# Amandaynzhou/MMT-PSM

Measured on AMD Instinct MI355X. Metric: imgs/sec (student+teacher step, 1000x1000, AUG_K=2), higher is better.
Workload: dtype f32

## Files before the change

### include/mmtpsm.h

```cpp
#ifndef MMTPSM_H
#define MMTPSM_H
#include <stdint.h>
#ifdef __cplusplus
extern "C" {
#endif

#define MMT_EINVAL (-22)

int mmt_version(void);

typedef struct {
  const float* feat[4];
  float* grad_feat[4];
  int H[4];
  int W[4];
  float scale[4];
  int num_levels;
  int N;
  int C;
} mmt_pyramid;

int mmt_roi_align_forward(const mmt_pyramid* pyr , const float* rois, const int32_t* levels,
                          int K, int PH, int PW, int sampling_ratio, float* out, void* stream);
int mmt_roi_align_forward_bf16(const mmt_pyramid* pyr , const float* rois, const int32_t* levels,
// ... 103 lines not shown
  const void* f16_guard_x;
  const void* f16_guard_dy;
  const void* w_src;
  const void* w_src_scale;
  int x_planes_layout;
  void* y_rb;
  long y_rb_stride;
  const float* y_rb_scale;
  void* y_amax_next;
  int x_planes_lag;
  int y_rb_rows;
} mmt_conv_args;

int mmt_conv_forward(const mmt_conv_args* a , void* stream);
int mmt_conv_variant(const mmt_conv_args* a );
int mmt_conv_ksplit(const mmt_conv_args* a );
int mmt_conv_wants_planes(const mmt_conv_args* a );
int mmt_set_conv_precision(int mode);
int mmt_amax(const float* x, long n, const float* rowscale, long inner, int rows, float* amax , void* stream);
int mmt_amax_stats(const float* x, long n, float* slot , void* stream);
int mmt_sum_stats(const float* a, const float* b, const float* c, const float* d, float* y, long n,
                  float* slot , void* stream);
int mmt_stats_combine(const float* const* slots , int n, float* out , void* stream);
int mmt_split_planes_f16(const float* x, void* planes, long plane_stride, long n, float scale, const float* amax ,
                         float* scale_out , float* amax_next ,
                         float* zero_slot , void* stream);
int mmt_pack_weight_f16(const float* w, void* planes, long plane_stride, int Cout, int K, float scale, const float* amax,
                        float* scale_out, void* stream);
int mmt_pack_weight_flipped_f16(const float* w, const float* scale, void* planes, long plane_stride, int Cout, int KH, int KW,
                                int Cin, const float* amax, float* scale_out, void* stream);
int mmt_conv3x3_strip_f16x2(const mmt_conv_args* a , const float* s_x , const float* s_w , void* stream);
int mmt_conv_forward_f16x2(const mmt_conv_args* a , const float* x_amax , const float* s_w , void* stream);
int mmt_get_conv_precision(void);
int mmt_stem_fused(const float* x, int N, int H, int W, const float* w_s2d, const void* w_planes, long w_plane_stride,
                   const float* s_w , const float* scale, const float* shift, const float* x_slot , float* y,
                   float* y_slot , void* stream);
int mmt_conv_wgrad_planes_splits(const mmt_conv_args* a );
int mmt_conv_wgrad_planes(const mmt_conv_args* a , const float* dy, const void* x_planes, long x_plane_stride,
                          const void* dy_planes, long dy_plane_stride, const float* s_x, const float* s_dy, const float* rowscale,
                          float* dw, float* dbias, float* workspace, void* stream);
typedef struct {
  void* fn;
  long a[16];
} mmt_call;
int mmt_replay(const mmt_call* calls , int n, int* failed_index );
int mmt_split_planes_f16_rb(const float* x, void* planes, long plane_stride, int rows, int W, int C, const float* amax,
                            float* scale_out, void* stream);
int mmt_conv_writes_rb(const mmt_conv_args* a );
typedef struct mmt_wgrad_job {
  mmt_conv_args a;
  const float* dy; const float* rowscale; float* dw; float* dbias;
  const void* x_planes; long x_plane_stride; const void* dy_planes; long dy_plane_stride; const float* s_x; const float* s_dy;
} mmt_wgrad_job;
int mmt_conv_wgrad_group_workspace(const mmt_wgrad_job* jobs , int n, long* floats_out );
int mmt_conv_wgrad_group(const mmt_wgrad_job* jobs , int n, float* workspace, long workspace_floats, void* stream);
int mmt_sum_stats_rb(const float* a, const float* b, const float* c, const float* d, float* y, int rows, int W, int C, float* slot,
                     void* planes, long plane_stride, const float* scale, float* amax_next, void* stream);
int mmt_rb_scales_update(float* state, int n, void* stream);
int mmt_conv_forward_pg(const mmt_conv_args* a , const float* s_x , const float* s_w , int tile_rows,
                        int ksplit, void* stream);
int mmt_conv_pg_plan(const mmt_conv_args* a , int* tile_rows, int* ksplit);
int mmt_conv_pg_wanted(const mmt_conv_args* a );
typedef struct { long src_off, dst_off; int Cout, K, unit0, pad; } mmt_pack_desc;
long mmt_packed_weight_elems(int Cout, int K);
int mmt_pack_weight(const float* w, void* planes, long plane_stride, int Cout, int K, void* stream);
int mmt_pack_weight_flipped(const float* w, const float* scale, void* planes, long plane_stride, int Cout, int KH, int KW,
// ... 110 lines not shown
```

### mmt-psm_amd/csrc/conv_igemm.hip

```cpp
#include <stdlib.h>
#include <map>
#include <mutex>
#include <type_traits>
#include "conv_shared.h"

namespace {

template <int BM, int BN, int WM, int WN>
__device__ __forceinline__ void conv_epilogue_stage(f32x16 (&acc)[BM / (32 * WM)][BN / (32 * WN)], float* lds,
                                                    const int lane, const int wm, const int wn) {
  constexpr int TM = BM / (32 * WM), TN = BN / (32 * WN);
  float* ct = lds;
  const int col_l = lane & 31, rq = lane >> 5;
#pragma unroll
  for (int a = 0; a < TM; a++)
#pragma unroll
    for (int b = 0; b < TN; b++)
#pragma unroll
      for (int r = 0; r < 16; r++) {
        const int row = (wm * TM + a) * 32 + (r & 3) + 8 * (r >> 2) + 4 * rq;
        ct[row * BN + (wn * TN + b) * 32 + col_l] = acc[a][b][r];
      }
}

// ... 125 lines not shown
            for (int e = 0; e < 4; e++) { const float av = e < nv ? fabsf(v[e]) : 0.f; amx = fmaxf(amx, av); asum += av; }
            acnt += (float)nv;
          }
          if (p.io & IO_Y) {
            unsigned short* yh = (unsigned short*)p.y + oidx[g];
            const unsigned lo = pk_bf16(v[0], v[1]), hi = pk_bf16(v[2], v[3]);
            if (vec) *(uint2*)yh = uint2{lo, hi};
            else { const unsigned short h4[4] = {(unsigned short)lo, (unsigned short)(lo >> 16), (unsigned short)hi, (unsigned short)(hi >> 16)};
                   for (int e = 0; e < nv; e++) yh[e] = h4[e]; }
            continue;
          }
          if (vec) *(f32x4*)(p.y + oidx[g]) = f32x4{v[0], v[1], v[2], v[3]};
          else for (int e = 0; e < nv; e++) p.y[oidx[g] + e] = v[e];
          if (p.ypl) {
            uint2 o[3];
            split4<3>(f32x4{v[0], v[1], v[2], v[3]}, o);
#pragma unroll
            for (int q = 0; q < 3; q++) *(uint2*)(p.ypl + q * p.ypl_stride + oidx[g]) = o[q];
          }
          if (p.yrb && m0 + r0 + (g0 + g) * RPP < p.yrb_M) rb_store4(p, rbg, m0 + r0 + (g0 + g) * RPP, c, f32x4{v[0], v[1], v[2], v[3]}, rbs);
        }
      }
    }
  }
  if (p.amax_out) {
    if (acc) { acc->amx = fmaxf(acc->amx, amx); acc->asum += asum; acc->acnt += acnt; }
    else conv_amax_commit(p, AmaxAcc{amx, asum, acnt}, blockIdx.x);
  }
}

template <int BM, int BN, int WM, int WN>
__device__ __forceinline__ void conv_epilogue(const ConvP& p, f32x16 (&acc)[BM / (32 * WM)][BN / (32 * WN)], float* lds,
                                              const int m0, const int n0, const int tid, const int lane,
                                              const int wm, const int wn, const int HoWo) {
  conv_epilogue_stage<BM, BN, WM, WN>(acc, lds, lane, wm, wn);
  __syncthreads();
  conv_epilogue_finish<BM, BN>(p, lds, m0, n0, tid, HoWo);
}

template <int BM, int BN, int WM, int WN>
__global__ __launch_bounds__(256, 2) void conv_fwd_kernel(const ConvP p) {
  constexpr int TM = BM / (32 * WM), TN = BN / (32 * WN);
  constexpr int NA = BM / 32, NB = BN / 32;
  extern __shared__ __attribute__((aligned(16))) float lds[];
  float* ldsA = lds;
  float* ldsB = lds + 2 * BM * 32;

  const int tid = threadIdx.x;
  const int lane = tid & 63;
  const int wave = __builtin_amdgcn_readfirstlane(tid >> 6);
  const int wm = wave / WN, wn = wave % WN;

  const int tiles_m = (p.M + BM - 1) / BM;
  const int tiles_n = (p.Cout + BN - 1) / BN;
  int bid = blockIdx.x;
  {
    const int nwg = tiles_m * tiles_n, q = nwg >> 3, r = nwg & 7, xcd = bid & 7, idx = bid >> 3;
    bid = (xcd < r ? xcd * (q + 1) : r * (q + 1) + (xcd - r) * q) + idx;
  }
  const int tile_m = bid / tiles_n, tile_n = bid % tiles_n;
  const int m0 = tile_m * BM, n0 = tile_n * BN;

  const int c4 = tid & 7;
  const int r8 = tid >> 3;
  unsigned abase[NA];
  int aih0[NA], aiw0[NA];
  bool aok[NA];
  const int HoWo = p.Ho * p.Wo;
#pragma unroll
  for (int j = 0; j < NA; j++) {
// ... 253 lines not shown
#pragma unroll
      for (int b = 0; b < TN; b++) fb[q][b] = *(const bf16x8*)(B + q * PB + b * 32 * 32);
    }
#pragma unroll
    for (int sum = 2 * (NS - 1) > NS - 1 ? NS - 1 : 0; sum >= 0; sum--)
#pragma unroll
      for (int qa = 0; qa <= sum; qa++) {
        const int qb = sum - qa;
        if (qa < NS && qb < NS) {
#pragma unroll
          for (int a = 0; a < TM; a++)
#pragma unroll
            for (int b = 0; b < TN; b++)
              acc[a][b] = __builtin_amdgcn_mfma_f32_32x32x16_bf16(fa[qa][a], fb[qb][b], acc[a][b], 0, 0, 0);
        }
      }
    if (kt + 1 < nkt) store_tile(buf ^ 1);
    __syncthreads();
  }
  conv_epilogue<BM, BN, WM, WN>(p, acc, lds, m0, n0, tid, lane, wm, wn, HoWo);
}

__device__ __attribute__((aligned(16))) const float g_zero16[4] = {0.f, 0.f, 0.f, 0.f};

__device__ __forceinline__ void dma16(const void* g, void* l) {
  __builtin_amdgcn_global_load_lds((const __attribute__((address_space(1))) void*)g, (lds_ptr_t)l, 16, 0, 0);
}

__device__ __forceinline__ void dma16_unseen(const void* g, void* l) {
#if defined(__HIP_DEVICE_COMPILE__)
  const unsigned la = __builtin_amdgcn_readfirstlane((unsigned)(unsigned long)(__attribute__((address_space(3))) char*)l);
  asm volatile("s_mov_b32 m0, %1\n\ts_nop 0\n\tglobal_load_lds_dwordx4 %0, off" ::"v"(g), "s"(la) : "m0", "memory");
#endif
}

template <int BM, int BN, int WM, int WN, int NS, int S, bool F16 = false>
__global__ __launch_bounds__(256, 2) void conv_fwd_glds_kernel(const ConvP p, const unsigned short* __restrict__ wpl,
                                                               const long wpl_stride, const int ksplit,
                                                               float* __restrict__ ws) {
  constexpr int TM = BM / (32 * WM), TN = BN / (32 * WN);
  constexpr int A_BYTES = BM * 64;
  constexpr int PB = BN * 32;
  constexpr int STAGE = A_BYTES + NS * PB;
  constexpr int NIA = BM / 64;
  constexpr int NIB_TOT = NS * BN / 32;
  constexpr int NIB = (NIB_TOT + 3) / 4;
  constexpr int NI = NIA + NIB;
  extern __shared__ __attribute__((aligned(16))) float lds[];
  char* const ring = (char*)lds;

  const int tid = threadIdx.x;
  const int lane = tid & 63;
  const int wave = __builtin_amdgcn_readfirstlane(tid >> 6);
  const int wm = wave / WN, wn = wave % WN;

  const int tiles_m = (p.M + BM - 1) / BM;
  const int tiles_n = (p.Cout + BN - 1) / BN;
  int bid = blockIdx.x;
  {
    const int nwg = tiles_m * tiles_n * ksplit, q = nwg >> 3, r = nwg & 7, xcd = bid & 7, idx = bid >> 3;
    bid = (xcd < r ? xcd * (q + 1) : r * (q + 1) + (xcd - r) * q) + idx;
  }
  const int ks = bid % ksplit;
  bid /= ksplit;
  const int tile_m = bid / tiles_n, tile_n = bid % tiles_n;
  const int m0 = tile_m * BM, n0 = tile_n * BN;
  const int HoWo = p.Ho * p.Wo;
  F16Guard guard = {};
  if constexpr (F16) guard = f16_guard_load(p.guard_x);
  unsigned abase[NIA];
  int aih0[NIA], aiw0[NIA], achunk[NIA];
  bool aok[NIA];
#pragma unroll
  for (int i = 0; i < NIA; i++) {
    const int row = (wave + 4 * i) * 16 + (lane >> 2);
    const int m = m0 + row;
    aok[i] = m < p.M;
    const int mm = aok[i] ? m : 0;
    const int img = mm / HoWo, rem = mm - img * HoWo;
    const int ho = rem / p.Wo, wo = rem - ho * p.Wo;
    aih0[i] = ho * p.stride - p.pad;
    aiw0[i] = wo * p.stride - p.pad;
    abase[i] = (unsigned)img * (unsigned)(p.H * p.W * p.Cin);
    achunk[i] = ((lane & 3) ^ ((row >> 2) & 3)) * 4;
  }
  const int nb32 = (p.Cout + 31) >> 5;
  const long kt_stride = (long)nb32 * 512;
  const unsigned short* bsrc[NIB];
  int bdst[NIB];
#pragma unroll
  for (int i = 0; i < NIB; i++) {
    const int t = (wave + 4 * i) % NIB_TOT;
    const int q = t / (BN / 32), rb = t % (BN / 32);
    int nb = n0 / 32 + rb;
    if (nb >= nb32) nb = nb32 - 1;
    bsrc[i] = wpl + q * wpl_stride + (long)nb * 512 + lane * 8;
    bdst[i] = A_BYTES + q * PB + rb * 1024;
  }
// ... 129 lines not shown
    __builtin_amdgcn_s_barrier();
    tap_next();
    filling = kt + S < nkt;
    const int kt_fill = min(kt + S, nkt - 1);
    constexpr int NM = TM * TN * (NS * (NS + 1) / 2);
    int j = 0, mi = 0;
#pragma unroll
    for (int sum = NS - 1; sum >= 0; sum--)
#pragma unroll
      for (int qa = 0; qa <= sum; qa++) {
        const int qb = sum - qa;
#pragma unroll
        for (int a = 0; a < TM; a++)
#pragma unroll
          for (int b = 0; b < TN; b++) {
            if constexpr (F16)
              acc[a][b] = __builtin_amdgcn_mfma_f32_32x32x16_f16(__builtin_bit_cast(f16x8, fa[qa][a]), __builtin_bit_cast(f16x8, fb[qb][b]), acc[a][b], 0, 0, 0);
            else
              acc[a][b] = __builtin_amdgcn_mfma_f32_32x32x16_bf16(fa[qa][a], fb[qb][b], acc[a][b], 0, 0, 0);
            j++;
#pragma unroll
            for (int r = 0; r < (NMICRO + NM - 1) / NM; r++)
              if (mi < (j * NMICRO + NM - 1) / NM) { micro(mi, kt_fill, stage_free, stage_next, fan, fbn); mi++; }
            __builtin_amdgcn_sched_barrier(0);
          }
      }
  };
#pragma unroll
  for (int t = 0; t < S - 1; t++) { filling = t < nkt; issue_all(min(t, nkt - 1), t); }
  if constexpr (F16) {
    if (f16_guard_bad(guard)) {
      asm volatile("s_waitcnt vmcnt(0)" ::: "memory");
      float* slab = ksplit > 1 ? ws + ((long)bid * ksplit + ks) * (BM * BN) : nullptr;
      conv_slow_tile(m0, BM, 0, BM, n0, BN, slab, ks != 0, tid, 256, blockIdx.x);
      return;
    }
  }
  wait_dma(S - 2);
  __builtin_amdgcn_s_barrier();
  filling = S - 1 < nkt;
  issue_all(min(S - 1, nkt - 1), S - 1);
  bf16x8 fa0[NS][TM], fb0[NS][TN], fa1[NS][TM], fb1[NS][TN];
  {
    const char* st = ring;
#pragma unroll
    for (int a = 0; a < TM; a++) { va[a][0] = *(const f32x4*)(st + aoff[a][0]); va[a][1] = *(const f32x4*)(st + aoff[a][1]); }
#pragma unroll
    for (int q = 0; q < NS; q++)
#pragma unroll
      for (int b = 0; b < TN; b++) fb0[q][b] = *(const bf16x8*)(st + boff + q * PB + b * 1024);
#pragma unroll
    for (int lvl = 0; lvl < SPL; lvl++)
#pragma unroll
      for (int f = 0; f < 2 * TM; f++) { if (lvl & 1) split_sub(f >> 1, f & 1); else split_cvt(f >> 1, f & 1, lvl >> 1); }
    pack_a(fa0);
  }
  int stage = 0;
  for (int kt = 0; kt < nkt; kt += 2) {
    const int s1 = stage == S - 1 ? 0 : stage + 1, s2 = s1 == S - 1 ? 0 : s1 + 1;
    step(kt, s1, stage, fa0, fb0, fa1, fb1);
    if (kt + 1 < nkt) step(kt + 1, s2, s1, fa1, fb1, fa0, fb0);
    stage = s2;
  }
  asm volatile("s_waitcnt vmcnt(0)" ::: "memory");
  __syncthreads();
  if (ksplit == 1) {
    if (!p.staged_epilogue && !p.io && !p.ypl && !p.mul && p.res_mode <= 1 && p.out_stride == 1 && (long)p.M * p.Cout * 4 < (1L << 31)) {
      const int mrow0 = m0 + wm * TM * 32 + 4 * (lane >> 5);
      conv_epilogue_direct<TM, TN>(p, acc, (unsigned)mrow0 * ((unsigned)p.Cout * 4u), p.M - mrow0, n0 + wn * TN * 32 + (lane & 31),
                                   (1 << (TM * TN)) - 1, lds + 64, wave, lane, tid, blockIdx.x);
      return;
    }
    conv_epilogue<BM, BN, WM, WN>(p, acc, lds, m0, n0, tid, lane, wm, wn, HoWo);
    return;
  }
  conv_epilogue_stage<BM, BN, WM, WN>(acc, lds, lane, wm, wn);
  __syncthreads();
  constexpr int TILE4 = BM * BN / 4;
  f32x4* slab = (f32x4*)ws + ((long)bid * ksplit + ks) * TILE4;
  const f32x4* ct4 = (const f32x4*)lds;
  for (int i = tid; i < TILE4; i += 256) slab[i] = ct4[i];
}

template <int BM, int BN, int WM, int WN, int NS, int S>
__global__ __launch_bounds__(256, 2) void conv_fwd_pp_kernel(const ConvP p, const int ksplit, float* __restrict__ ws) {
  constexpr int TM = BM / (32 * WM), TN = BN / (32 * WN);
  constexpr int PA = BM * 32, PB = BN * 32;
  constexpr int A_BYTES = NS * PA;
  constexpr int STAGE = A_BYTES + NS * PB;
  constexpr int NIA_TOT = NS * BM / 32, NIB_TOT = NS * BN / 32;
  constexpr int NIA = (NIA_TOT + 3) / 4, NIB = (NIB_TOT + 3) / 4, NI = NIA + NIB;
  static_assert(BM / 32 == 4 || BM / 32 == 2, "row blocks per wave");
  extern __shared__ __attribute__((aligned(16))) float lds[];
  char* const ring = (char*)lds;

  const int tid = threadIdx.x;
  const int lane = tid & 63;
  const int wave = __builtin_amdgcn_readfirstlane(tid >> 6);
  const int wm = wave / WN, wn = wave % WN;

  const int tiles_m = (p.M + BM - 1) / BM;
  const int tiles_n = (p.Cout + BN - 1) / BN;
  int bid = blockIdx.x;
  {
    const int nwg = tiles_m * tiles_n * ksplit, q = nwg >> 3, r = nwg & 7, xcd = bid & 7, idx = bid >> 3;
    bid = (xcd < r ? xcd * (q + 1) : r * (q + 1) + (xcd - r) * q) + idx;
// ... 1015 lines not shown
  }
}

template <int NS>
int launch_split_variant(int variant, const ConvP& p, hipStream_t s) {
  switch (variant) {
    case 1: return launch_split<128, 128, 2, 2, NS>(p, s);
    case 3: return launch_split<128, 64, 2, 2, NS>(p, s);
    default: return launch_split<64, 64, 2, 2, NS>(p, s);
  }
}

}

namespace mmtconv {
static int g_precision = -1;
int precision() {
  if (g_precision < 0) {
    g_precision = getenv("MMT_CONV_PRECISION") ? atoi(getenv("MMT_CONV_PRECISION")) : 3;
    if (g_precision < 0 || g_precision > 3) g_precision = 3;
  }
  return g_precision;
}
}

extern "C" int mmt_set_conv_precision(int mode) {
  if (mode < 0 || mode > 3) return MMT_EINVAL;
  mmtconv::g_precision = mode;
  return 0;
}

extern "C" int mmt_get_conv_precision(void) { return precision(); }

extern "C" int mmt_conv3x3_strip_f16x2(const mmt_conv_args* a, const float* s_x, const float* s_w, void* stream) {
  ConvP p;
  int e = fill(p, a);
  if (e) return e;
  if (!p.y || !p.xpl || !p.wpl || !s_x || !s_w || p.io || p.ypl) return MMT_EINVAL;
  p.f16_sx = s_x; p.f16_sw = s_w;
  const int tw = strip_tw(p);
  if (!tw) return MMT_EINVAL;
  const int ksplit = strip_ksplit(p, tw);
  constexpr int NS = 2;
  hipStream_t s = (hipStream_t)stream;
  SplitWs w{nullptr, nullptr};
  if (ksplit > 1) {
    w = split_workspace(s);
    if (!w.ws) return MMT_EINVAL;
  }
  const int tiles = p.N * (p.Ho * p.Wo / 256) * mmt_cdiv(p.Cout, 128);
  auto go = [&](auto kern, int TW) {
    const int R = 256 / TW, SW = TW + 32;
    const size_t ring = (size_t)2 * (NS * R * SW * 32 + 3 * NS * 128 * 32), epi = (size_t)256 * 128 * sizeof(float);
    const size_t lds = ring > epi ? ring : epi;
    const hipError_t er = hipFuncSetAttribute((const void*)kern, hipFuncAttributeMaxDynamicSharedMemorySize, (int)lds);
    if (er != hipSuccess) return (int)er;
    hipLaunchKernelGGL(kern, dim3(tiles * ksplit), dim3(512), lds, s, p, ksplit | strip_korder(p), w.ws);
    return 0;
  };
  if (tw == 128) e = go(conv3x3_strip_kernel<128, NS, true>, 128);
  else e = go(conv3x3_strip_kernel<64, NS, true>, 64);
  if (e) return e;
  MMT_LAUNCH_CHECK();
  if (ksplit > 1) {
    launch_finish<256, 128>(p, tiles, ksplit, w.ws, s);
    MMT_LAUNCH_CHECK();
// ... 8 lines not shown
  return true;
}
extern "C" int mmt_conv_writes_rb(const mmt_conv_args* a) {
  ConvP p;
  if (fill(p, a) || precision() != 3 || p.io) return 0;
  p.f16_ax = 1;
  p.f16_sx = p.f16_sw = (const float*)16;
  return rb_epilogue_ok(p) ? 1 : 0;
}
extern "C" int mmt_conv_forward_f16x2(const mmt_conv_args* a, const float* x_amax, const float* s_w, void* stream) {
  ConvP p;
  int e = fill(p, a);
  if (e) return e;
  if (!p.y || !p.wpl || !x_amax || !s_w || p.io || p.ypl || p.xpl_rb || (p.Cin & 15) || ((size_t)p.wpl & 15) || (p.wpl_stride & 7)) return MMT_EINVAL;
  if (p.M == 0 || p.Cout == 0) return 0;
  const int variant = pick_variant(p);
  if (variant == 0) return MMT_EINVAL;
  p.f16_sx = x_amax; p.f16_sw = s_w; p.f16_ax = 1;
  hipStream_t s = (hipStream_t)stream;
  if (p.yrb && !rb_epilogue_ok(p)) return MMT_EINVAL;
  if (c64_shape(p)) return launch_c64(p, s);
  if (rows_shape(p, true)) {
    if (p.mask) {
      if (p.Cin == 64) return launch_rows<4, 2, true, true>(p, s);
      if (p.Cin == 128) return launch_rows<8, 2, true, true>(p, s);
      return launch_rows<16, 2, true, true>(p, s);
    }
    if (p.Cin == 64) return launch_rows<4, 2, true>(p, s);
    if (p.Cin == 128) return launch_rows<8, 2, true>(p, s);
    return launch_rows<16, 2, true>(p, s);
  }
  const int ksplit = pick_ksplit(p);
  constexpr int S = 3;
  auto go = [&](auto kern, int BM, int BN, int ks) -> int {
    const int tiles = mmt_cdiv(p.M, BM) * mmt_cdiv(p.Cout, BN) * ks;
    SplitWs w{nullptr, nullptr};
    if (ks > 1) {
      w = split_workspace(s);
      if (!w.ws || tiles > 1024) return MMT_EINVAL;
    }
    const size_t ring = (size_t)S * (BM * 64 + 2 * BN * 32), epi = (size_t)BM * BN * sizeof(float);
    const size_t lds = ring > epi ? ring : epi;
    if (lds > 65536) {
      const hipError_t er = hipFuncSetAttribute((const void*)kern, hipFuncAttributeMaxDynamicSharedMemorySize, (int)lds);
      if (er != hipSuccess) return (int)er;
    }
    hipLaunchKernelGGL(kern, dim3(tiles), dim3(256), lds, s, p, p.wpl, p.wpl_stride, ks, w.ws);
    if (ks > 1)
      launch_finish<128, 128>(p, tiles / ks, ks, w.ws, s);
    return 0;
  };
#define MMT_GLDS_GO(SS)                                                                                      \
  do {                                                                                                       \
    if (ksplit > 1) e = go(conv_fwd_glds_kernel<128, 128, 4, 1, 2, SS, true>, 128, 128, ksplit);            \
    else if (variant == 1) e = go(conv_fwd_glds_kernel<128, 128, 4, 1, 2, SS, true>, 128, 128, 1);          \
    else if (variant == 3) e = go(conv_fwd_glds_kernel<128, 64, 4, 1, 2, SS, true>, 128, 64, 1);            \
    else e = go(conv_fwd_glds_kernel<64, 64, 2, 2, 2, SS, true>, 64, 64, 1);                                \
  } while (0)
  MMT_GLDS_GO(3);
#undef MMT_GLDS_GO
  if (e) return e;
  MMT_LAUNCH_CHECK();
  return 0;
}

static int pick_variant(const ConvP& p) {
  if (p.Cout <= 32) return 0;
  constexpr int lowk = 256;
  constexpr int lowv = 3;
  if (p.K <= lowk) return (p.Cout >= 64 && (long)mmt_cdiv(p.M, 128) * mmt_cdiv(p.Cout, 64) >= 768) ? lowv : 2;
  const long t128 = (long)mmt_cdiv(p.M, 128) * mmt_cdiv(p.Cout, 128);
  constexpr int t128min = 256;
  if (t128 >= t128min && p.Cout > 64) return 1;
  constexpr int mid = 1;
  const long t12864 = (long)mmt_cdiv(p.M, 128) * mmt_cdiv(p.Cout, 64);
  if (mid && t12864 >= 256 && p.Cout >= 64) return 3;
  return 2;
}

extern "C" int mmt_conv_variant(const mmt_conv_args* a) {
  ConvP p;
  int e = fill(p, a);
  if (e) return e;
  const int v = pick_variant(p);
// ... 52 lines not shown
```

### mmt-psm_amd/csrc/conv_wgrad.hip

```cpp
#include <stdlib.h>
#include <type_traits>
#include "conv_shared.h"

namespace {

template <bool FAST>
__global__ __launch_bounds__(256) void conv_wgrad_kernel(const ConvP p, const float* __restrict__ dy,
                                                         const float* __restrict__ rowscale,
                                                         float* __restrict__ dw, int m_per_split,
                                                         float* __restrict__ ws) {
  constexpr int BM = 128, BN = 128;
  extern __shared__ __attribute__((aligned(16))) float lds[];
  float* ldsA = lds;
  float* ldsB = lds + 2 * 32 * 128;
  const int tid = threadIdx.x, lane = tid & 63;
  const int wave = __builtin_amdgcn_readfirstlane(tid >> 6);
  const int wm = wave >> 1, wn = wave & 1;
  const int co0 = blockIdx.y * BM, n0 = blockIdx.x * BN;
  const int NP = p.KH * p.KW * p.Cin;
  const int ms = blockIdx.z * m_per_split;
  const int me = min(p.M, ms + m_per_split);
  if (ms >= me) return;

  const int c4 = tid & 31;
// ... 334 lines not shown
        const int ho = rem / pk->Wo, wo = rem - ho * pk->Wo;
        const int ih = ho * pk->stride - pk->pad + kh, iw = wo * pk->stride - pk->pad + kw;
        if ((unsigned)ih < (unsigned)pk->H && (unsigned)iw < (unsigned)pk->W)
          acc = fmaf(dy[(long)m * pk->Cout + co], x[((long)(img * pk->H + ih) * pk->W + iw) * pk->Cin + ci], acc);
      }
    }
    ct[o] = acc * s;
  }
  if (dbias && tid < 128 && co0 + tid < pk->Cout) {
    float b = 0.f;
    for (int m = ms; m < me; m++) b += dy[(long)m * pk->Cout + co0 + tid];
    atomicAdd(dbias + co0 + tid, b);
  }
}

template <int NS, int MODE, bool VEC4, int BF = 0, bool F16 = false>
__device__ __forceinline__ void conv_wgrad_pipe_body(const ConvP& p_in, const float* __restrict__ dy,
                                                     const float* __restrict__ rowscale,
                                                     float* __restrict__ dw, int m_per_split,
                                                     float* __restrict__ ws, float* __restrict__ dbias,
                                                     const int tx, const int ty, const int tz, const int lin) {
  constexpr int PL = 2 * 128 * 16;
  constexpr int STAGE = 2 * NS * PL;
  extern __shared__ __attribute__((aligned(16))) float lds[];
  char* const ring = (char*)lds;
  const int tid = threadIdx.x, lane = tid & 63;
  const int wave = __builtin_amdgcn_readfirstlane(tid >> 6);
  const int wm = wave >> 1, wn = wave & 1;
  int bx, by, bz;
  {
    const int nwg = tx * ty * tz;
    const int q = nwg >> 3, r = nwg & 7, xcd = lin & 7, idx = lin >> 3;
    const int id = (xcd < r ? xcd * (q + 1) : r * (q + 1) + (xcd - r) * q) + idx;
    bx = id % tx;
    const int t = id / tx;
    by = t % ty;
    bz = t / ty;
  }
  const ConvP p = p_in;
  const int co0 = by * 128, n0 = bx * 128;
  const int NP = p.KH * p.KW * p.Cin;
  const int ms = bz * m_per_split;
  const int me = min(p.M, ms + m_per_split);
  if (ms >= me) return;
  const int HoWo = p.Ho * p.Wo;
  F16Guard guard_x = {}, guard_dy = {};
  if constexpr (F16) { guard_x = f16_guard_load(p.guard_x); guard_dy = f16_guard_load(p.guard_dy); }

  const bool roleB = wave >= 2;
  const int cq = (wave & 1) * 16 + (lane & 15);
  const int pg = lane >> 4;
  const int ch = (roleB ? n0 : co0) + cq * 4;
  bool col_ok;
  int bkh = 0, bkw = 0, bci = 0;
  if (roleB) {
    col_ok = ch < NP;
    if (col_ok) { const int tap = ch / p.Cin; bci = ch - tap * p.Cin; bkh = tap / p.KW; bkw = tap - bkh * p.KW; }
  } else {
    col_ok = ch < p.Cout;
  }
  const int woff = (pg >> 1) * 2048 + cq * 16 + (pg & 1) * 8 + (roleB ? NS * PL : 0);
  int r_img[4], r_ho[4], r_wo[4];
#pragma unroll
  for (int j = 0; j < 4; j++) {
    const int m = ms + pg * 4 + j;
    r_img[j] = m / HoWo;
    const int rem = m - r_img[j] * HoWo;
    r_ho[j] = rem / p.Wo;
    r_wo[j] = rem - r_ho[j] * p.Wo;
  }
// ... 631 lines not shown
```

### mmt-psm_amd/maskrcnn_benchmark/_hip.py

```python
import ctypes
import weakref
import os
import threading as _threading

import torch

_HERE = os.path.dirname(os.path.abspath(__file__))
LIB_PATH = os.path.join(os.path.dirname(_HERE), "libmmtpsm.so")

c_void_p, c_int, c_float, c_double, c_int64 = ctypes.c_void_p, ctypes.c_int, ctypes.c_float, ctypes.c_double, ctypes.c_int64


class Pyramid(ctypes.Structure):
    _fields_ = [("feat", c_void_p * 4), ("grad_feat", c_void_p * 4), ("H", c_int * 4), ("W", c_int * 4),
                ("scale", c_float * 4), ("num_levels", c_int), ("N", c_int), ("C", c_int)]


class ConvArgs(ctypes.Structure):
    _fields_ = [("x", c_void_p), ("w", c_void_p), ("scale", c_void_p), ("shift", c_void_p), ("res", c_void_p),
                ("mask", c_void_p), ("mul", c_void_p), ("y", c_void_p),
                ("N", c_int), ("H", c_int), ("W", c_int), ("Cin", c_int), ("Cout", c_int), ("KH", c_int),
                ("KW", c_int), ("stride", c_int), ("pad", c_int), ("Ho", c_int), ("Wo", c_int),
                ("relu", c_int), ("res_mode", c_int), ("out_stride", c_int), ("out_H", c_int), ("out_W", c_int),
                ("mask_scale", c_float), ("w_planes", c_void_p), ("w_plane_stride", ctypes.c_long),
# ... 40 lines not shown
                ("key_scratch", c_void_p)]


class MgdTeachers(ctypes.Structure):
    _fields_ = [("t", c_void_p * 8), ("flip", c_int * 8), ("nt", c_int)]


class MgdStudents(ctypes.Structure):
    _fields_ = [("s", c_void_p * 4), ("mirror", c_int * 4), ("ns", c_int)]


_SIGS = {
    "mmt_version": [],
    "mmt_roi_align_forward": [ctypes.POINTER(Pyramid), c_void_p, c_void_p, c_int, c_int, c_int, c_int, c_void_p, c_void_p],
    "mmt_roi_align_forward_bf16": [ctypes.POINTER(Pyramid), c_void_p, c_void_p, c_int, c_int, c_int, c_int, c_void_p, c_void_p],
    "mmt_roi_align_backward": [ctypes.POINTER(Pyramid), c_void_p, c_void_p, c_int, c_int, c_int, c_int, c_void_p, c_void_p],
    "mmt_roi_align_backward_dense": [ctypes.POINTER(Pyramid), c_void_p, c_void_p, c_int, c_int, c_int, c_int, c_void_p, c_void_p],
    "mmt_nms_batched": [c_void_p, c_void_p, c_int, c_int, c_float, c_void_p, c_void_p, c_void_p, c_void_p],
    "mmt_resample_u8": [c_void_p, c_void_p, c_int, c_int, c_int, c_int, c_void_p, c_void_p, c_int, c_void_p],
    "mmt_aug_views": [c_void_p, c_int, c_int, c_int, c_void_p, c_void_p, c_void_p, c_void_p, c_int, ctypes.POINTER(c_float),
                      c_void_p, ctypes.c_long, c_int, c_int, c_void_p],
    "mmt_aug_erase": [c_void_p, ctypes.c_long, c_int, c_int, c_void_p, c_void_p, c_void_p, c_int, ctypes.POINTER(c_float),
                      c_void_p],
    "mmt_roi_format_levels": [c_void_p, c_void_p, c_int, c_float, c_float, c_float, c_int, c_int, c_void_p, c_void_p, c_void_p],
    "mmt_relation_reg_labels": [c_void_p, c_void_p, c_void_p, c_void_p, c_int, c_int, c_int, ctypes.POINTER(c_float), c_int, c_void_p, c_void_p],
    "mmt_match_targets": [c_void_p, c_void_p, c_void_p, c_void_p, c_void_p, c_void_p, c_int, c_int, c_int, c_int, c_float,
                          c_float, c_int, c_float, c_float, c_float, c_float, c_void_p, c_void_p, c_void_p, c_void_p, c_void_p,
                          c_void_p],
    "mmt_conv_forward": [ctypes.POINTER(ConvArgs), c_void_p],
    "mmt_conv_variant": [ctypes.POINTER(ConvArgs)],
    "mmt_conv_ksplit": [ctypes.POINTER(ConvArgs)],
    "mmt_set_conv_precision": [ctypes.c_int],
    "mmt_get_conv_precision": [],
    "mmt_pack_weight": [c_void_p, c_void_p, ctypes.c_long, c_int, c_int, c_void_p],
    "mmt_rpn_topk": [c_void_p, c_int, c_int, c_int, c_void_p, c_void_p],
    "mmt_rpn_gather_decode": [ctypes.POINTER(RpnSelectArgs), c_void_p],
    "mmt_rpn_post_select": [ctypes.POINTER(RpnPostArgs), c_void_p],
    "mmt_sample_fg_bg": [c_void_p, c_int, c_void_p, c_void_p, c_int, c_int, c_int, c_void_p, c_void_p, c_void_p, c_void_p],
    "mmt_box_decode": [c_void_p, c_void_p, c_int, c_int, c_float, c_float, c_float, c_float, c_float, c_void_p, c_void_p, c_int,
                       c_void_p, c_void_p],
    "mmt_split_planes": [c_void_p, c_void_p, ctypes.c_long, ctypes.c_long, c_void_p],
    "mmt_conv_wants_planes": [ctypes.POINTER(ConvArgs)],
    "mmt_pack_weights": [c_void_p, c_void_p, ctypes.c_long, c_void_p, c_void_p, c_int, c_void_p],
    "mmt_pack_weights_flipped": [c_void_p, c_void_p, c_int, c_void_p],
    "mmt_pack_weights_f16": [c_void_p, c_void_p, ctypes.c_long, c_void_p, c_void_p, c_int, c_int, c_void_p, c_void_p],
    "mmt_pack_weights_flipped_f16": [c_void_p, c_void_p, c_int, c_int, c_void_p, c_void_p],
    "mmt_pack_weight_flipped": [c_void_p, c_void_p, c_void_p, ctypes.c_long, c_int, c_int, c_int, c_int, c_void_p],
    "mmt_conv_wgrad_splits": [ctypes.POINTER(ConvArgs)],
    "mmt_conv_wgrad": [ctypes.POINTER(ConvArgs), c_void_p, c_void_p, c_void_p, c_void_p, c_void_p, c_void_p],
    "mmt_colsum": [c_void_p, c_int, c_int, c_void_p, c_void_p],
    "mmt_weight_flip_transpose": [c_void_p, c_void_p, c_void_p, c_int, c_int, c_int, c_int, c_void_p],
    "mmt_maxpool3x3s2": [c_void_p, c_void_p, c_int, c_int, c_int, c_int, c_int, c_int, c_void_p],
    "mmt_amax": [c_void_p, ctypes.c_long, c_void_p, ctypes.c_long, c_int, c_void_p, c_void_p],
    "mmt_amax_stats": [c_void_p, ctypes.c_long, c_void_p, c_void_p],
    "mmt_det_postprocess": [c_void_p, c_void_p, c_void_p, c_void_p, c_int, c_int, c_float, c_float, c_int, c_void_p,
                            c_void_p, c_void_p, c_void_p, c_void_p, c_void_p],
    "mmt_position_embedding": [c_void_p, c_int, c_int, c_int, c_void_p, c_void_p, c_void_p],
    "mmt_sample_fg_bg_wide": [c_void_p, c_int, c_void_p, c_void_p, c_int, c_int, c_int, c_int, c_void_p, c_void_p, c_void_p, c_void_p,
                              c_void_p],
    "mmt_rpn_loss": [c_void_p, c_void_p, c_void_p, c_void_p, c_void_p, c_void_p, ctypes.c_long, c_float, c_void_p, c_void_p, c_void_p,
                     c_void_p, c_void_p],
    "mmt_box_loss": [c_void_p, c_void_p, c_void_p, c_void_p, c_int, c_int, c_void_p, c_void_p, c_void_p, c_void_p],
    "mmt_box_loss_rows": [c_void_p, c_void_p, c_void_p, c_void_p, c_int, c_int, c_void_p, c_void_p, c_void_p, c_void_p, c_void_p],
    "mmt_relation_attention_fwd": [c_void_p, c_void_p, c_void_p, c_void_p, c_void_p, c_int, c_int, c_int, c_int, c_int, c_int, c_float,
                                   c_void_p, c_void_p, c_void_p],
    "mmt_relation_attention_bwd": [c_void_p, c_void_p, c_void_p, c_void_p, c_void_p, c_void_p, c_int, c_int, c_int, c_int, c_int, c_float,
# ... 568 lines not shown
        raise NotImplementedError("MMT_DETERMINISTIC=1 with MMT_BF16_STORAGE=1: deterministic mode is not offered with bf16 activation storage")
    _det_torch(True)


def _refuse_unordered(kernel, what):
    if _DET:
        raise NotImplementedError("%s is not offered in deterministic mode: %s adds into its destination with float atomics and has "
                                  "no ordered form yet; set_deterministic(False)" % (what, kernel))


def lib():
    global _lib
    if _lib is None:
        if not os.path.exists(LIB_PATH):
            raise RuntimeError(
                "libmmtpsm.so not found at %s: build it with `make -C mmt-psm_amd/csrc` "
                "(or python -c 'import __graft_entry__ as g; g.build()'); there is no fallback path" % LIB_PATH)
        L = ctypes.CDLL(LIB_PATH)
        for name, args in _SIGS.items():
            f = getattr(L, name)
            f.restype = c_int
            f.argtypes = args
        if _DET:
            L.mmt_set_deterministic(1)
        _lib = _LibProxy(L)
    return _lib


def _lib_raw():
    return lib()._L


_NO_RECORD = frozenset(("mmt_conv_wants_planes", "mmt_conv_pg_wanted", "mmt_conv_writes_rb", "mmt_conv_wgrad_group_workspace", "mmt_conv_variant", "mmt_conv_ksplit", "mmt_conv_pg_plan",
                        "mmt_conv_wgrad_splits", "mmt_get_conv_precision", "mmt_packed_weight_elems", "mmt_set_conv_precision", "mmt_set_deterministic", "mmt_get_deterministic"))
LAYOUT_EPOCH = [0]
LAUNCH_PLANS = os.environ.get("MMT_LAUNCH_PLANS", "1") != "0"
_LP_SLOTS = 512
_LP_MAX = 4
_LAUNCH_PLANS = {}
_LP_LOCK = _threading.Lock()


class _LibProxy(object):

    def __init__(self, L):
        self._L = L

    def __getattr__(self, name):
        f = getattr(self._L, name)
        if name in _NO_RECORD:
            w = f
        else:
            def w(*args, _f=f):
                rec = getattr(_TLS, "rec", None)
                if rec is not None:
                    rec.calls.append((_f, args))
                return _f(*args)
        self.__dict__[name] = w
        return w


class _Call(ctypes.Structure):
    _fields_ = [("fn", c_void_p), ("a", ctypes.c_long * 16)]


C_REPLAY = os.environ.get("MMT_C_REPLAY", "1") != "0"

# ... 1035 lines not shown
                                             _stream()), "mmt_pack_weight_flipped")
        if flat is not None:
            flat.register("bf16_dgrad", w, scale, planes)
    return planes


def pack_weights(base, planes, descs, unit_desc, n_units):
    _check(lib().mmt_pack_weights(base.data_ptr(), planes.data_ptr(), planes.stride(0), descs.data_ptr(),
                                  unit_desc.data_ptr(), n_units, _stream()), "mmt_pack_weights")


def _weight_planes(w, a):
    if get_conv_precision() == 0 or (w.shape[1] & 15) or w.shape[0] <= 32:
        return None, None
    flat, pl = _flat_form(w, "bf16")
    if pl is None:
        flat, pl = None, pack_weight(w)
    a.w_planes, a.w_plane_stride = pl.data_ptr(), pl.stride(0)
    return pl, flat


_PREC = None


def set_conv_precision(mode):
    global PLANES_EPOCH, _PREC
    _check(lib().mmt_set_conv_precision(int(mode)), "mmt_set_conv_precision")
    _PREC = lib().mmt_get_conv_precision()
    PLANES_EPOCH += 1
    _PLAN_EPOCH[0] += 1
    _PLAN.clear()


def get_conv_precision():
    global _PREC
    if _PREC is None:
        _PREC = lib().mmt_get_conv_precision()
    return _PREC


def wgrad_prepare(x, dy):
    if F16X2 and x.dtype == torch.float32 and dy.dtype == torch.float32 and x.numel() >= WGRAD_F16_MIN_ELEMS and get_conv_precision() == 3:
        _amax_of(nhwc(x))
        _amax_of(nhwc(dy))


def _wgrad_stats(x, dy, dw, passes):
    ax, ad = _recorded(x), _recorded(dy)
    if passes and x.numel() >= WGRAD_F16_MIN_ELEMS:
        if ax is None:
            ax = _amax_of(x)
        if ad is None:
            ad = _amax_of(dy)
    if ax is None or ad is None or not (_site_ok(("wgx", dw.data_ptr()), x) and _site_ok(("wgd", dw.data_ptr()), dy)):
        return None
    return ax, ad


def _wgrad_planes(x, dy, st=None):
    xr, dr = _rb_of(x), _rb_of(dy)
    if xr is None or dr is None or xr[4] is not None or dr[4] is not None:
        return None
    lag = (1 if xr[3] == "epi" else 0) | (2 if dr[3] == "epi" else 0)
    if st is not None and lag and (_guard(st[0]) is None or _guard(st[1]) is None):
        return None
    return xr, dr, lag
# ... 621 lines not shown
```

Baseline: 123.1.

## Add row-feed 1x1 conv kernel with register-fed A and deep LDS ring for B

Adds a specialised forward kernel for 1x1 stride-1 convolutions with large Cin. It loads activation rows directly into registers and splits them to f16 on the fly, while weight planes stream into a deeper LDS ring through buffer-to-LDS DMA, with loads interleaved between MFMA instructions. This aims to cut LDS traffic and hide memory latency on the large-K GEMMs. It also changes tile rasterisation (XCD-aware ordering that favours N-major when Cout exceeds M) for both forward and wgrad, and threads a logical block id through the amax stats. The cost is more code paths and a different accumulation and tile order, and it runs by default.

```diff
diff --git a/include/mmtpsm.h b/include/mmtpsm.h
--- a/include/mmtpsm.h
+++ b/include/mmtpsm.h
@@ -159,6 +159,7 @@
 int mmt_conv3x3_strip_f16x2(const mmt_conv_args* a , const float* s_x , const float* s_w , void* stream);
 int mmt_conv_forward_f16x2(const mmt_conv_args* a , const float* x_amax , const float* s_w , void* stream);
 int mmt_get_conv_precision(void);
+int mmt_set_row_feed(int on);
 int mmt_stem_fused(const float* x, int N, int H, int W, const float* w_s2d, const void* w_planes, long w_plane_stride,
                    const float* s_w , const float* scale, const float* shift, const float* x_slot , float* y,
                    float* y_slot , void* stream);
diff --git a/mmt-psm_amd/csrc/conv_igemm.hip b/mmt-psm_amd/csrc/conv_igemm.hip
--- a/mmt-psm_amd/csrc/conv_igemm.hip
+++ b/mmt-psm_amd/csrc/conv_igemm.hip
@@ -181,10 +181,13 @@
 template <int BM, int BN, int WM, int WN>
 __device__ __forceinline__ void conv_epilogue(const ConvP& p, f32x16 (&acc)[BM / (32 * WM)][BN / (32 * WN)], float* lds,
                                               const int m0, const int n0, const int tid, const int lane,
-                                              const int wm, const int wn, const int HoWo) {
+                                              const int wm, const int wn, const int HoWo, const int lin = -1) {
   conv_epilogue_stage<BM, BN, WM, WN>(acc, lds, lane, wm, wn);
   __syncthreads();
-  conv_epilogue_finish<BM, BN>(p, lds, m0, n0, tid, HoWo);
+  if (lin < 0) { conv_epilogue_finish<BM, BN>(p, lds, m0, n0, tid, HoWo); return; }
+  AmaxAcc a;
+  conv_epilogue_finish<BM, BN>(p, lds, m0, n0, tid, HoWo, &a);
+  if (p.amax_out) conv_amax_commit(p, a, lin);
 }
 
 template <int BM, int BN, int WM, int WN>
@@ -504,6 +507,29 @@
   const unsigned la = __builtin_amdgcn_readfirstlane((unsigned)(unsigned long)(__attribute__((address_space(3))) char*)l);
   asm volatile("s_mov_b32 m0, %1\n\ts_nop 0\n\tglobal_load_lds_dwordx4 %0, off" ::"v"(g), "s"(la) : "m0", "memory");
 #endif
+}
+
+struct TileId { int ks, tile_m, tile_n, tile, lin; };
+__device__ __forceinline__ TileId glds_tile_of(const ConvP& p, const int tiles_m, const int tiles_n, const int ksplit) {
+  const int tiles = tiles_m * tiles_n, nwg = tiles * ksplit, q = nwg >> 3, r = nwg & 7;
+  const int xcd = blockIdx.x & 7, idx = blockIdx.x >> 3;
+  const int bid = (xcd < r ? xcd * (q + 1) : r * (q + 1) + (xcd - r) * q) + idx;
+  TileId t;
+  t.ks = ksplit > 1 ? bid / tiles : 0;
+  const int rr = bid - t.ks * tiles;
+  const bool planes_larger = p.Cout > p.M;
+  if (planes_larger) { t.tile_n = rr / tiles_m; t.tile_m = rr - t.tile_n * tiles_m; }
+  else { t.tile_m = rr / tiles_n; t.tile_n = rr - t.tile_m * tiles_n; }
+  t.tile = t.tile_m * tiles_n + t.tile_n;
+  t.lin = blockIdx.x;
+  if (planes_larger || ksplit > 1) {
+    const int old = t.tile * ksplit + t.ks, head = r * (q + 1);
+    int ox, oi;
+    if (old < head) { ox = old / (q + 1); oi = old - ox * (q + 1); }
+    else { ox = r + (old - head) / q; oi = (old - head) - (ox - r) * q; }
+    t.lin = oi * 8 + ox;
+  }
+  return t;
 }
 
 template <int BM, int BN, int WM, int WN, int NS, int S, bool F16 = false>
@@ -528,14 +554,8 @@
 
   const int tiles_m = (p.M + BM - 1) / BM;
   const int tiles_n = (p.Cout + BN - 1) / BN;
-  int bid = blockIdx.x;
-  {
-    const int nwg = tiles_m * tiles_n * ksplit, q = nwg >> 3, r = nwg & 7, xcd = bid & 7, idx = bid >> 3;
-    bid = (xcd < r ? xcd * (q + 1) : r * (q + 1) + (xcd - r) * q) + idx;
-  }
-  const int ks = bid % ksplit;
-  bid /= ksplit;
-  const int tile_m = bid / tiles_n, tile_n = bid % tiles_n;
+  const TileId tile_id = glds_tile_of(p, tiles_m, tiles_n, ksplit);
+  const int ks = tile_id.ks, bid = tile_id.tile, tile_m = tile_id.tile_m, tile_n = tile_id.tile_n, lin = tile_id.lin;
   const int m0 = tile_m * BM, n0 = tile_n * BN;
   const int HoWo = p.Ho * p.Wo;
   F16Guard guard = {};
@@ -731,7 +751,7 @@
     if (f16_guard_bad(guard)) {
       asm volatile("s_waitcnt vmcnt(0)" ::: "memory");
       float* slab = ksplit > 1 ? ws + ((long)bid * ksplit + ks) * (BM * BN) : nullptr;
-      conv_slow_tile(m0, BM, 0, BM, n0, BN, slab, ks != 0, tid, 256, blockIdx.x);
+      conv_slow_tile(m0, BM, 0, BM, n0, BN, slab, ks != 0, tid, 256, lin);
       return;
     }
   }
@@ -767,10 +787,203 @@
     if (!p.staged_epilogue && !p.io && !p.ypl && !p.mul && p.res_mode <= 1 && p.out_stride == 1 && (long)p.M * p.Cout * 4 < (1L << 31)) {
       const int mrow0 = m0 + wm * TM * 32 + 4 * (lane >> 5);
       conv_epilogue_direct<TM, TN>(p, acc, (unsigned)mrow0 * ((unsigned)p.Cout * 4u), p.M - mrow0, n0 + wn * TN * 32 + (lane & 31),
-                                   (1 << (TM * TN)) - 1, lds + 64, wave, lane, tid, blockIdx.x);
+                                   (1 << (TM * TN)) - 1, lds + 64, wave, lane, tid, lin);
       return;
     }
-    conv_epilogue<BM, BN, WM, WN>(p, acc, lds, m0, n0, tid, lane, wm, wn, HoWo);
+    conv_epilogue<BM, BN, WM, WN>(p, acc, lds, m0, n0, tid, lane, wm, wn, HoWo, lin);
+    return;
+  }
+  conv_epilogue_stage<BM, BN, WM, WN>(acc, lds, lane, wm, wn);
+  __syncthreads();
+  constexpr int TILE4 = BM * BN / 4;
+  f32x4* slab = (f32x4*)ws + ((long)bid * ksplit + ks) * TILE4;
+  const f32x4* ct4 = (const f32x4*)lds;
+  for (int i = tid; i < TILE4; i += 256) slab[i] = ct4[i];
+}
+
+#ifndef MMT_ROW_FEED_DEPTH
+#define MMT_ROW_FEED_DEPTH 6
+#endif
+template <int BN, int S>
+__global__ __launch_bounds__(256, 2) void conv_fwd_rowfeed_kernel(const ConvP p, const unsigned short* __restrict__ wpl,
+                                                                  const long wpl_stride, const int ksplit,
+                                                                  float* __restrict__ ws) {
+  constexpr int BM = 128, WM = 4, WN = 1, NS = 2, TM = 1, TN = BN / 32;
+  constexpr int PB = BN * 32;
+  constexpr int STAGE = NS * PB;
+  constexpr int NIB_TOT = NS * BN / 32;
+  constexpr int NIB = (NIB_TOT + 3) / 4;
+  constexpr int NI = 2 + NIB;
+  constexpr int U = (S & 1) ? 2 * S : S;
+  static_assert(S >= 3 && S <= 8 && (S - 2) * NI < 64 && S * STAGE <= BM * BN * 4, "ring depth");
+  extern __shared__ __attribute__((aligned(16))) float lds[];
+  char* const ring = (char*)lds;
+
+  const int tid = threadIdx.x;
+  const int lane = tid & 63;
+  const int wave = __builtin_amdgcn_readfirstlane(tid >> 6);
+  const int wm = wave, wn = 0;
+
+  const int tiles_m = (p.M + BM - 1) / BM;
+  const int tiles_n = (p.Cout + BN - 1) / BN;
+  const TileId tile_id = glds_tile_of(p, tiles_m, tiles_n, ksplit);
+  const int ks = tile_id.ks, bid = tile_id.tile, lin = tile_id.lin;
+  const int m0 = tile_id.tile_m * BM, n0 = tile_id.tile_n * BN;
+  const int HoWo = p.Ho * p.Wo;
+  const F16Guard guard = f16_guard_load(p.guard_x);
+  const int nkt_all = p.K >> 4;
+  const int kt0 = (int)((long)ks * nkt_all / ksplit), nkt = (int)((long)(ks + 1) * nkt_all / ksplit) - kt0;
+  const int nb32 = (p.Cout + 31) >> 5;
+  const long kt_stride = (long)nb32 * 512;
+  const __amdgpu_buffer_rsrc_t rw = __builtin_amdgcn_make_buffer_rsrc((void*)(wpl + (long)kt0 * kt_stride), 0, (int)0x80000000u, 0x00020000);
+  unsigned bvo[NIB];
+  int bdst[NIB];
+#pragma unroll
+  for (int i = 0; i < NIB; i++) {
+    const int t = (wave + 4 * i) % NIB_TOT;
+    const int q = t / (BN / 32), rb = t % (BN / 32);
+    int nb = n0 / 32 + rb;
+    if (nb >= nb32) nb = nb32 - 1;
+    bvo[i] = (unsigned)(q * wpl_stride + (long)nb * 512) * 2u + (unsigned)lane * 16u;
+    bdst[i] = q * PB + rb * 1024;
+  }
+  const int lr = lane & 31, kh2 = lane >> 5;
+  const __amdgpu_buffer_rsrc_t rx = __builtin_amdgcn_make_buffer_rsrc((void*)p.x, 0, (int)((long)p.M * p.Cin * 4), 0x00020000);
+  const int mrow = m0 + wave * 32 + lr;
+  const unsigned arow = mrow < p.M ? ((unsigned)mrow * (unsigned)p.Cin + 16u * (unsigned)kt0 + 8u * (unsigned)kh2) * 4u : 0x80000000u;
+  f32x4 qa[S][2];
+  bool filling = true;
+  auto load_a = [&](int slot, int h, int kt) {
+    const unsigned off = (filling ? arow : 0x80000000u) + (unsigned)kt * 64u + (unsigned)h * 16u;
+    qa[slot][h] = __builtin_bit_cast(f32x4, __builtin_amdgcn_raw_buffer_load_b128(rx, (int)off, 0, 0));
+  };
+  auto dma_b = [&](int i, int kt, int stage) {
+    __builtin_amdgcn_raw_ptr_buffer_load_lds(rw, (lds_ptr_t)(ring + stage * STAGE + bdst[i]), 16, (int)(filling ? bvo[i] : 0x80000000u),
+                                             (int)((unsigned)kt * (unsigned)kt_stride * 2u), 0, 0);
+  };
+  auto issue_all = [&](int slot, int kt) {
+    load_a(slot, 0, kt);
+    load_a(slot, 1, kt);
+#pragma unroll
+    for (int i = 0; i < NIB; i++) dma_b(i, kt, slot);
+  };
+  const int boff = lr * 32 + (((kh2 ^ (lr >> 3)) & 1) << 4);
+
+  f32x16 acc[TM][TN];
+#pragma unroll
+  for (int b = 0; b < TN; b++)
+#pragma unroll
+    for (int r = 0; r < 16; r++) acc[0][b][r] = 0.f;
+
+  unsigned ua[2][2];
+  uint2 oa[2][NS];
+  const float f16_sx = f16_scale_of(*p.f16_sx);
+  auto split_cvt = [&](f32x4& v, int h, int q) {
+    if (q == 0) v *= f16_sx;
+    ua[h][0] = __builtin_bit_cast(unsigned, f16x2{(_Float16)v[0], (_Float16)v[1]});
+    ua[h][1] = __builtin_bit_cast(unsigned, f16x2{(_Float16)v[2], (_Float16)v[3]});
+    oa[h][q] = uint2{ua[h][0], ua[h][1]};
+  };
+  auto split_sub = [&](f32x4& v, int h) {
+    const f16x2 h0 = __builtin_bit_cast(f16x2, ua[h][0]), h1 = __builtin_bit_cast(f16x2, ua[h][1]);
+    v[0] -= (float)h0[0]; v[1] -= (float)h0[1]; v[2] -= (float)h1[0]; v[3] -= (float)h1[1];
+  };
+  auto pack_a = [&](bf16x8 (&fa)[NS]) {
+#pragma unroll
+    for (int q = 0; q < NS; q++) {
+      const uint4 u = {oa[0][q].x, oa[0][q].y, oa[1][q].x, oa[1][q].y};
+      fa[q] = __builtin_bit_cast(bf16x8, u);
+    }
+  };
+  constexpr int SPL = 2 * NS - 1;
+  constexpr int M_LD = 2 + NIB, M_RB = NS * TN, M_SPLIT = 2 * SPL;
+  constexpr int NMICRO = M_LD + M_RB + M_SPLIT + 1;
+  bf16x8 fa[2][NS], fb[2][NS][TN];
+  auto micro = [&](const int J, int idx, int kt) {
+    const int SF = J % S, SN = (J + 1) % S, PN = (J + 1) & 1;
+    if (idx < 2) { load_a(SF, idx, kt + S); return; }
+    idx -= 2;
+    if (idx < NIB) { dma_b(idx, kt + S, SF); return; }
+    idx -= NIB;
+    const char* st = ring + SN * STAGE;
+    if (idx < M_RB) { const int q = idx / TN, b = idx % TN; fb[PN][q][b] = *(const bf16x8*)(st + boff + q * PB + b * 1024); return; }
+    idx -= M_RB;
+    if (idx < M_SPLIT) {
+      const int lvl = idx >> 1, h = idx & 1;
+      if (lvl & 1) split_sub(qa[SN][h], h); else split_cvt(qa[SN][h], h, lvl >> 1);
+      return;
+    }
+    pack_a(fa[PN]);
+  };
+  auto wait_dma = [&]() {
+    asm volatile("s_waitcnt vmcnt(%0) lgkmcnt(0)" ::"n"((S - 2) * NI) : "memory");
+  };
+  auto step = [&](const int J, const int kt) {
+    const int PC = J & 1;
+    wait_dma();
+    __builtin_amdgcn_s_barrier();
+    filling = kt + S < nkt;
+    constexpr int NM = TN * (NS * (NS + 1) / 2);
+    int j = 0, mi = 0;
+#pragma unroll
+    for (int sum = NS - 1; sum >= 0; sum--)
+#pragma unroll
+      for (int qa_ = 0; qa_ <= sum; qa_++) {
+        const int qb = sum - qa_;
+#pragma unroll
+        for (int b = 0; b < TN; b++) {
+          acc[0][b] = __builtin_amdgcn_mfma_f32_32x32x16_f16(__builtin_bit_cast(f16x8, fa[PC][qa_]), __builtin_bit_cast(f16x8, fb[PC][qb][b]), acc[0][b], 0, 0, 0);
+          j++;
+#pragma unroll
+          for (int r = 0; r < (NMICRO + NM - 1) / NM; r++)
+            if (mi < (j * NMICRO + NM - 1) / NM) { micro(J, mi, kt); mi++; }
+          __builtin_amdgcn_sched_barrier(0);
+        }
+      }
+  };
+#pragma unroll
+  for (int t = 0; t < S - 1; t++) { filling = t < nkt; issue_all(t, t); }
+  if (f16_guard_bad(guard)) {
+    asm volatile("s_waitcnt vmcnt(0)" ::: "memory");
+    float* slab = ksplit > 1 ? ws + ((long)bid * ksplit + ks) * (BM * BN) : nullptr;
+    conv_slow_tile(m0, BM, 0, BM, n0, BN, slab, ks != 0, tid, 256, lin);
+    return;
+  }
+  wait_dma();
+  __builtin_amdgcn_s_barrier();
+  filling = S - 1 < nkt;
+  issue_all(S - 1, S - 1);
+  {
+#pragma unroll
+    for (int q = 0; q < NS; q++)
+#pragma unroll
+      for (int b = 0; b < TN; b++) fb[0][q][b] = *(const bf16x8*)(ring + boff + q * PB + b * 1024);
+#pragma unroll
+    for (int lvl = 0; lvl < SPL; lvl++)
+#pragma unroll
+      for (int h = 0; h < 2; h++) { if (lvl & 1) split_sub(qa[0][h], h); else split_cvt(qa[0][h], h, lvl >> 1); }
+    pack_a(fa[0]);
+  }
+  int kt = 0;
+  for (; kt + U <= nkt; kt += U) {
+#pragma unroll
+    for (int j = 0; j < U; j++) step(j, kt + j);
+  }
+#pragma unroll
+  for (int j = 0; j < U; j++) {
+    if (kt + j >= nkt) break;
+    step(j, kt + j);
+  }
+  asm volatile("s_waitcnt vmcnt(0)" ::: "memory");
+  __syncthreads();
+  if (ksplit == 1) {
+    if (!p.staged_epilogue && !p.io && !p.ypl && !p.mul && p.res_mode <= 1 && p.out_stride == 1 && (long)p.M * p.Cout * 4 < (1L << 31)) {
+      const int mrow0 = m0 + wm * TM * 32 + 4 * (lane >> 5);
+      conv_epilogue_direct<TM, TN>(p, acc, (unsigned)mrow0 * ((unsigned)p.Cout * 4u), p.M - mrow0, n0 + wn * TN * 32 + (lane & 31),
+                                   (1 << (TM * TN)) - 1, lds + 64, wave, lane, tid, lin);
+      return;
+    }
+    conv_epilogue<BM, BN, WM, WN>(p, acc, lds, m0, n0, tid, lane, wm, wn, HoWo, lin);
     return;
   }
   conv_epilogue_stage<BM, BN, WM, WN>(acc, lds, lane, wm, wn);
@@ -1852,6 +2065,16 @@
 
 extern "C" int mmt_get_conv_precision(void) { return precision(); }
 
+static int g_row_feed = 1;
+extern "C" int mmt_set_row_feed(int on) {
+  g_row_feed = on ? 1 : 0;
+  return 0;
+}
+static bool rowfeed_shape(const ConvP& p) {
+  return g_row_feed && p.KH == 1 && p.KW == 1 && p.stride == 1 && p.pad == 0 && p.Ho == p.H && p.Wo == p.W && (p.Cin & 31) == 0 &&
+         p.Cin >= 512 && (long)p.M * p.Cin * 4 < (1L << 31) && p.wpl_stride < (1L << 28);
+}
+
 extern "C" int mmt_conv3x3_strip_f16x2(const mmt_conv_args* a, const float* s_x, const float* s_w, void* stream) {
   ConvP p;
   int e = fill(p, a);
@@ -1926,6 +2149,7 @@
   }
   const int ksplit = pick_ksplit(p);
   constexpr int S = 3;
+  const bool rowfeed = (ksplit > 1 || variant == 3) && rowfeed_shape(p);
   auto go = [&](auto kern, int BM, int BN, int ks) -> int {
     const int tiles = mmt_cdiv(p.M, BM) * mmt_cdiv(p.Cout, BN) * ks;
     SplitWs w{nullptr, nullptr};
@@ -1933,7 +2157,7 @@
       w = split_workspace(s);
       if (!w.ws || tiles > 1024) return MMT_EINVAL;
     }
-    const size_t ring = (size_t)S * (BM * 64 + 2 * BN * 32), epi = (size_t)BM * BN * sizeof(float);
+    const size_t ring = rowfeed ? (size_t)MMT_ROW_FEED_DEPTH * (2 * BN * 32) : (size_t)S * (BM * 64 + 2 * BN * 32), epi = (size_t)BM * BN * sizeof(float);
     const size_t lds = ring > epi ? ring : epi;
     if (lds > 65536) {
       const hipError_t er = hipFuncSetAttribute((const void*)kern, hipFuncAttributeMaxDynamicSharedMemorySize, (int)lds);
@@ -1944,6 +2168,15 @@
       launch_finish<128, 128>(p, tiles / ks, ks, w.ws, s);
     return 0;
   };
+  if (rowfeed) {
+    typedef void (*rowfeed_kernel_t)(const ConvP, const unsigned short*, const long, const int, float*);
+    const rowfeed_kernel_t k128 = conv_fwd_rowfeed_kernel<128, MMT_ROW_FEED_DEPTH>, k64 = conv_fwd_rowfeed_kernel<64, MMT_ROW_FEED_DEPTH>;
+    if (ksplit > 1) e = go(k128, 128, 128, ksplit);
+    else e = go(k64, 128, 64, 1);
+    if (e) return e;
+    MMT_LAUNCH_CHECK();
+    return 0;
+  }
 #define MMT_GLDS_GO(SS)                                                                                      \
   do {                                                                                                       \
     if (ksplit > 1) e = go(conv_fwd_glds_kernel<128, 128, 4, 1, 2, SS, true>, 128, 128, ksplit);            \
diff --git a/mmt-psm_amd/csrc/conv_wgrad.hip b/mmt-psm_amd/csrc/conv_wgrad.hip
--- a/mmt-psm_amd/csrc/conv_wgrad.hip
+++ b/mmt-psm_amd/csrc/conv_wgrad.hip
@@ -390,10 +390,17 @@
     const int nwg = tx * ty * tz;
     const int q = nwg >> 3, r = nwg & 7, xcd = lin & 7, idx = lin >> 3;
     const int id = (xcd < r ? xcd * (q + 1) : r * (q + 1) + (xcd - r) * q) + idx;
-    bx = id % tx;
-    const int t = id / tx;
-    by = t % ty;
-    bz = t / ty;
+    if (tz < 8 && p_in.KH * p_in.KW * p_in.Cin > p_in.Cout) {
+      by = id % ty;
+      const int t = id / ty;
+      bx = t % tx;
+      bz = t / tx;
+    } else {
+      bx = id % tx;
+      const int t = id / tx;
+      by = t % ty;
+      bz = t / ty;
+    }
   }
   const ConvP p = p_in;
   const int co0 = by * 128, n0 = bx * 128;
diff --git a/mmt-psm_amd/maskrcnn_benchmark/_hip.py b/mmt-psm_amd/maskrcnn_benchmark/_hip.py
--- a/mmt-psm_amd/maskrcnn_benchmark/_hip.py
+++ b/mmt-psm_amd/maskrcnn_benchmark/_hip.py
@@ -96,6 +96,7 @@
     "mmt_conv_ksplit": [ctypes.POINTER(ConvArgs)],
     "mmt_set_conv_precision": [ctypes.c_int],
     "mmt_get_conv_precision": [],
+    "mmt_set_row_feed": [ctypes.c_int],
     "mmt_pack_weight": [c_void_p, c_void_p, ctypes.c_long, c_int, c_int, c_void_p],
     "mmt_rpn_topk": [c_void_p, c_int, c_int, c_int, c_void_p, c_void_p],
     "mmt_rpn_gather_decode": [ctypes.POINTER(RpnSelectArgs), c_void_p],
@@ -730,7 +731,8 @@
 
 
 _NO_RECORD = frozenset(("mmt_conv_wants_planes", "mmt_conv_pg_wanted", "mmt_conv_writes_rb", "mmt_conv_wgrad_group_workspace", "mmt_conv_variant", "mmt_conv_ksplit", "mmt_conv_pg_plan",
-                        "mmt_conv_wgrad_splits", "mmt_get_conv_precision", "mmt_packed_weight_elems", "mmt_set_conv_precision", "mmt_set_deterministic", "mmt_get_deterministic"))
+                        "mmt_conv_wgrad_splits", "mmt_get_conv_precision", "mmt_packed_weight_elems", "mmt_set_conv_precision", "mmt_set_deterministic", "mmt_get_deterministic",
+                        "mmt_set_row_feed"))
 LAYOUT_EPOCH = [0]
 LAUNCH_PLANS = os.environ.get("MMT_LAUNCH_PLANS", "1") != "0"
 _LP_SLOTS = 512
@@ -1832,6 +1834,11 @@
     _PLAN.clear()
 
 
+def set_row_feed(on):
+    if lib().mmt_set_row_feed(1 if on else 0) != 0:
+        raise RuntimeError("mmt_set_row_feed failed")
+
+
 def get_conv_precision():
     global _PREC
     if _PREC is None:
```

Measured after the change: 123.2, median of 2. About the same (+0.1%).
